# steineggerlab/unicore

Hardware: AMD Instinct MI355X
Metric: 3Di alignments/sec (cluster path) (higher is better)
Workload: dtype u16

## Files before the change

unicore_amd/csrc/uc_sw_pk_impl.hpp:

```cpp
#pragma once
#include <hip/hip_runtime.h>

#include "uc_device.h"
#include "uc_sw_impl.hpp"

namespace uc {

constexpr int SW_PK_OVF = 0x7C00 - 256;

typedef uint16_t u16x2_t __attribute__((ext_vector_type(2)));
typedef uint32_t u32x4_u __attribute__((ext_vector_type(4), aligned(4)));
typedef uint32_t u32x2_u __attribute__((ext_vector_type(2), aligned(4)));
typedef const uint32_t __attribute__((address_space(4))) *sw_cu32p;
__device__ __forceinline__ u16x2_t pk_v(uint32_t x) { return __builtin_bit_cast(u16x2_t, x); }
__device__ __forceinline__ uint32_t pk_u(u16x2_t v) { return __builtin_bit_cast(uint32_t, v); }
__device__ __forceinline__ uint32_t pk_add_sat(uint32_t a, uint32_t b) { return pk_u(__builtin_elementwise_add_sat(pk_v(a), pk_v(b))); }
__device__ __forceinline__ uint32_t pk_sub_sat(uint32_t a, uint32_t b) { return pk_u(__builtin_elementwise_sub_sat(pk_v(a), pk_v(b))); }
__device__ __forceinline__ uint32_t pk_max(uint32_t a, uint32_t b) { return pk_u(__builtin_elementwise_max(pk_v(a), pk_v(b))); }
__device__ __forceinline__ uint32_t pk_min(uint32_t a, uint32_t b) {
    uint32_t r;
    asm("v_pk_min_u16 %0, %1, %2" : "=v"(r) : "v"(a), "v"(b));
    return r;
}
__device__ __forceinline__ uint32_t pk_max3(uint32_t a, uint32_t b, uint32_t c) {
    uint32_t r;
    asm("v_pk_maximum3_f16 %0, %1, %2, %3" : "=v"(r) : "v"(a), "v"(b), "v"(c));
    return r;
}
__device__ __forceinline__ uint32_t pk_max3_s(uint32_t a, uint32_t b, uint32_t c) {
    uint32_t r;
    asm("v_pk_maximum3_f16 %0, %1, %2, %3" : "=v"(r) : "v"(a), "v"(b), "s"(c));
    return r;
}
__device__ __forceinline__ uint32_t pk_max_s(uint32_t a, uint32_t c) {
    uint32_t r;
    asm("v_pk_max_u16 %0, %1, %2" : "=v"(r) : "v"(a), "s"(c));
    return r;
}
__device__ __forceinline__ uint32_t add3_s(uint32_t a, uint32_t b, uint32_t c) {
    uint32_t r;
    asm("v_add3_u32 %0, %1, %2, %3" : "=v"(r) : "v"(a), "v"(b), "s"(c));
    return r;
}
constexpr uint32_t SW_PK_BIAS = 128u * 0x10001u;
constexpr uint32_t SW_PK_UNBIAS = 0u - SW_PK_BIAS;
static_assert(SW_PK_UNBIAS == 0xFF7FFF80u, "the packed -128");

constexpr int SW_MQ_SLOTS = 128;

template <int G, int R, int MODE, int NW, int K = 1>
__global__ void __launch_bounds__(NW * 64) sw_pk_kernel(const SwArgs a) {
    constexpr bool TBB = MODE == 7;
    constexpr uint32_t HB = TBB ? 0u : SW_PK_BIAS;
    constexpr bool KNOWN = MODE == 4 || MODE == 6;
    constexpr int BASE = KNOWN ? MODE - 4 : (TBB ? 0 : MODE);
    constexpr bool TRACK = BASE != 1 && !TBB, MASK = BASE == 2 || TBB, REVQ = BASE != 0, REVT = BASE == 2;
    constexpr int RW = (R + 3) / 4, BW = RW | 1, RSW = G * BW, NT = NW * 64;
    static_assert(R % 2 == 0 && R <= 32, "R must be even, <= 32");
    extern __shared__ __attribute__((aligned(16))) uint32_t lds[];
    static_assert(K == 1 || (K <= 4 && G < 64 && !TBB), "several tasks per workgroup: G < 64, not MODE 7");
    constexpr int PB = 2 * SW_NLET * RSW;
    uint32_t *P3 = lds, *PA = lds + SW_NLET * RSW;
    uint32_t *slot_ctr = lds + K * PB;
    [[maybe_unused]] uint32_t *tinfo = slot_ctr + 4, *sstep = tinfo + 4 * K;
    [[maybe_unused]] uint8_t *stab = (uint8_t *)(sstep + SW_MQ_SLOTS);

    const SwTask task = a.tasks[K * blockIdx.x];
    const int tid = threadIdx.x, lane = tid & 63;
    const int g = lane % G;
    const uint32_t qoff = a.db.off[task.q];
    const int lq = (int)a.db.len[task.q];
    const uint32_t open2 = (uint32_t)a.open * 0x10001u, ext2 = (uint32_t)a.ext * 0x10001u, bias2 = 128u * 0x10001u;
    const uint32_t nslots = (task.count + 1) >> 1;

    for (int idx = tid; idx < SW_NLET * G * RW; idx += NT) {
        const int c = idx / (G * RW), rem = idx % (G * RW), gg = rem / RW, k = rem % RW;
        uint32_t w3 = 0, wa = 0;
#pragma unroll
        for (int b = 0; b < 4; b++) {
            const int row = gg * R + 4 * k + b;
            if (row < lq && c < 21 && 4 * k + b < R) {
                const int qi = REVQ ? lq - 1 - row : row;
                const int q3 = a.db.s3[qoff + qi], qa = a.db.sa[qoff + qi];
                w3 |= (uint32_t)(a.db.S3[q3 * 21 + c] + 64) << (8 * b);
                wa |= (uint32_t)(a.db.SA[qa * 21 + c] + 64) << (8 * b);
            }
        }
        P3[c * RSW + gg * BW + k] = w3;
        PA[c * RSW + gg * BW + k] = wa;
    }
    if constexpr (K > 1) {
        const uint32_t task0 = (uint32_t)K * blockIdx.x, nk = min((uint32_t)K, a.n_tasks - task0);
        uint32_t base[K + 1];
        base[0] = 0; base[1] = nslots;
        if (tid == 0) { tinfo[0] = task.begin; tinfo[1] = task.count; tinfo[2] = (uint32_t)lq; }
#pragma unroll
        for (int t = 1; t < K; t++) {
            base[t + 1] = base[t];
            if ((uint32_t)t < nk) {
                const SwTask tk = a.tasks[task0 + t];
                const uint32_t qofft = a.db.off[tk.q];
                const int lqt = (int)a.db.len[tk.q];
                for (int idx = tid; idx < SW_NLET * G * RW; idx += NT) {
                    const int c = idx / (G * RW), rem = idx % (G * RW), gg = rem / RW, k = rem % RW;
                    uint32_t w3 = 0, wa = 0;
#pragma unroll
                    for (int b = 0; b < 4; b++) {
                        const int row = gg * R + 4 * k + b;
                        if (row < lqt && c < 21 && 4 * k + b < R) {
                            const int qi = REVQ ? lqt - 1 - row : row;
                            const int q3 = a.db.s3[qofft + qi], qa = a.db.sa[qofft + qi];
                            w3 |= (uint32_t)(a.db.S3[q3 * 21 + c] + 64) << (8 * b);
                            wa |= (uint32_t)(a.db.SA[qa * 21 + c] + 64) << (8 * b);
                        }
                    }
                    P3[t * PB + c * RSW + gg * BW + k] = w3;
                    PA[t * PB + c * RSW + gg * BW + k] = wa;
                }
                base[t + 1] += (tk.count + 1) >> 1;
                if (tid == 0) { tinfo[4 * t] = tk.begin; tinfo[4 * t + 1] = tk.count; tinfo[4 * t + 2] = (uint32_t)lqt; }
            }
        }
        const uint32_t mq_slots = min(base[K], (uint32_t)SW_MQ_SLOTS);
        if (tid == 0) tinfo[3] = mq_slots;
        for (uint32_t e = tid; e < mq_slots; e += NT) {
            uint32_t t = 0;
#pragma unroll
            for (int j = 1; j < K; j++) t += e >= base[j] ? 1u : 0u;
            uint32_t eb = 0;
#pragma unroll
            for (int j = 1; j < K; j++) eb = t == (uint32_t)j ? base[j] : eb;
            const SwTask tk = a.tasks[task0 + t];
            const uint32_t i = e - eb, pA = tk.begin + 2 * i, pB = pA + (2 * i + 1 < tk.count ? 1u : 0u);
            const int la = REVT ? a.pte[pA] + 1 : (int)a.db.len[a.pt[pA]], lb = REVT ? a.pte[pB] + 1 : (int)a.db.len[a.pt[pB]];
            sstep[e] = ((uint32_t)((max(la, lb) + G) & ~1) << 8) | (t << 6) | i;
        }
    }
    if (tid == 0) *slot_ctr = 0;
    __syncthreads();
    if constexpr (K > 1) {
        const uint32_t mq_slots = tinfo[3];
        for (uint32_t e = tid; e < mq_slots; e += NT) {
            const uint32_t v = sstep[e], s = v >> 8;
            uint32_t rank = 0;
            for (uint32_t j = 0; j < mq_slots; j++) {
                const uint32_t sj = sstep[j] >> 8;
                rank += (sj > s || (sj == s && j < e)) ? 1u : 0u;
            }
            stab[rank] = (uint8_t)(v & 0xffu);
        }
        __syncthreads();
    }

    uint32_t H[R], E[R], rowbest[(TRACK && !KNOWN) ? R : 1];
    uint32_t mskA[MASK ? RW : 1], mskB[MASK ? RW : 1];
    uint32_t best = HB, Hlast = HB, prevHup = HB, fout = 0;
    int colA = -1, colB = -1;
    [[maybe_unused]] uint32_t knownA = 0, knownB = 0;
    [[maybe_unused]] int key2A = 0x7fffffff, key2B = 0x7fffffff;
    uint32_t gA = 0, gB = 0, toffA = 0, toffB = 0;
    [[maybe_unused]] unsigned long long tbA = 0, tbB = 0;
    [[maybe_unused]] int tsaA = 0, tsbA = 0, tsaB = 0, tsbB = 0;
    [[maybe_unused]] uint32_t trowA = 0, trowB = 0, tslotA = 0, tslotB = 0;
    int tlenA = 0, tlenB = 0, rowoffA = 0, rowoffB = 0;
    bool vB = false, active = false;
    int lst = 0, nst = 0;
    uint32_t c1 = 0, cin = 0;
    struct RawLetters { uint32_t a3, aa, b3, ba; } r2 = {0, 0, 0, 0};
    uint32_t nA3[RW], nAa[RW], nB3[RW], nBa[RW];
    [[maybe_unused]] const uint16_t *ltA = nullptr, *ltB = nullptr;

    auto issue_letters = [&](int st) -> RawLetters {
        RawLetters r;
        if constexpr (G == 64) {
            const int ia = max(min(st, tlenA - 1), 0), ib = max(min(st, tlenB - 1), 0);
            const uint32_t pa = toffA + (uint32_t)(REVT ? max(tlenA - 1 - ia, 0) : ia);
            const uint32_t pb_ = toffB + (uint32_t)(REVT ? max(tlenB - 1 - ib, 0) : ib);
            auto ld = [&](const uint8_t *base, uint32_t p) -> uint32_t {
                const sw_cu32p w = (sw_cu32p)(uintptr_t)(base + (p & ~3u));
                return (*w >> (8u * (p & 3u))) & 0xffu;
            };
            r.a3 = ld(a.db.s3, pa); r.aa = ld(a.db.sa, pa); r.b3 = ld(a.db.s3, pb_); r.ba = ld(a.db.sa, pb_);
        } else {
            const uint32_t ia = REVT ? (uint32_t)max(tlenA - st, 0) : (uint32_t)min(st, tlenA);
            const uint32_t ib = REVT ? (uint32_t)max(tlenB - st, 0) : (uint32_t)min(st, tlenB);
            r.a3 = ltA[ia]; r.b3 = ltB[ib];
            r.aa = 0; r.ba = 0;
        }
        return r;
    };
    auto pack_letters = [&](const RawLetters &r, int st) -> uint32_t {
        if constexpr (G == 64) {
            const uint32_t ca_ = st < tlenA ? (r.a3 | (r.aa << 8)) : SW_PADPACK;
            const uint32_t cb_ = st < tlenB ? (r.b3 | (r.ba << 8)) : SW_PADPACK;
            return ca_ | (cb_ << 16);
        } else if constexpr (TBB) {
            return (st < tlenA ? r.a3 : SW_PADPACK) | ((st < tlenB ? r.b3 : SW_PADPACK) << 16);
        } else {
            return r.a3 | (r.b3 << 16);
        }
    };
    uint32_t off3 = (uint32_t)(g * BW) * 4u, offa = (uint32_t)(SW_NLET * RSW + g * BW) * 4u;
    asm volatile("" : "+v"(off3), "+v"(offa));
    auto fetch_profile = [&]() __attribute__((always_inline)) {
        const char *l8 = (const char *)lds;
        const uint32_t *pA3 = (const uint32_t *)(l8 + (cin & 0xff) * (RSW * 4) + off3), *pAa = (const uint32_t *)(l8 + ((cin >> 8) & 0xff) * (RSW * 4) + offa);
        const uint32_t *pB3 = (const uint32_t *)(l8 + ((cin >> 16) & 0xff) * (RSW * 4) + off3), *pBa = (const uint32_t *)(l8 + (cin >> 24) * (RSW * 4) + offa);
#pragma unroll
        for (int k = 0; k < RW; k++) { nA3[k] = pA3[k]; nAa[k] = pAa[k]; nB3[k] = pB3[k]; nBa[k] = pBa[k]; }
    };

    auto start_slot = [&]() {
        uint32_t idx = 0;
        if (g == 0) idx = atomicAdd(slot_ctr, 1u);
        if constexpr (G == 64) idx = (uint32_t)__builtin_amdgcn_readfirstlane((int)idx);
        else idx = (uint32_t)__shfl((int)idx, lane - g, 64);
        if constexpr (K == 1) active = idx < nslots;
        else active = idx < tinfo[3];
        if (!active) return;
        [[maybe_unused]] uint32_t mq_begin = 0, mq_count = 0;
        [[maybe_unused]] int mq_lq = 0;
        if constexpr (K > 1) {
            const uint32_t code = stab[idx], t = code >> 6;
            idx = code & 63u;
            mq_begin = tinfo[4 * t]; mq_count = tinfo[4 * t + 1]; mq_lq = (int)tinfo[4 * t + 2];
            off3 = (t * PB + (uint32_t)(g * BW)) * 4u;
            offa = off3 + (uint32_t)(SW_NLET * RSW) * 4u;
        }
        const uint32_t iA = 2 * idx, iB = iA + 1;
        vB = iB < (K == 1 ? task.count : mq_count);
        gA = (K == 1 ? task.begin : mq_begin) + iA;
        gB = (K == 1 ? task.begin : mq_begin) + (vB ? iB : iA);
        const uint32_t tA = a.pt[gA], tB = a.pt[gB];
        toffA = a.db.off[tA]; toffB = a.db.off[tB];
        tlenA = REVT ? a.pte[gA] + 1 : (int)a.db.len[tA];
        tlenB = vB ? (REVT ? a.pte[gB] + 1 : (int)a.db.len[tB]) : 0;
        if constexpr (TBB) {
            toffA += (uint32_t)a.pts[gA]; toffB += (uint32_t)a.pts[gB];
            tlenA = a.pte[gA] - a.pts[gA] + 1;
            tlenB = vB ? a.pte[gB] - a.pts[gB] + 1 : 0;
            tbA = a.tboff[gA]; tbB = a.tboff[gB];
            const int qsA = a.pqs[gA], qeA = a.pqe[gA], qsB = a.pqs[gB], qeB = a.pqe[gB];
            {
                constexpr int RBc = 4 * RW;
                const TbBand bA = tb_band_of(qsA, qeA, tlenA, G, R, a.tb_band), bB = tb_band_of(qsB, qeB, vB ? tlenB : 1, G, R, a.tb_band);
                const bool fullA = bA.nl >= G, fullB = bB.nl >= G;
                tsaA = fullA ? 0 : g * (R + 1) - bA.dhi; tsbA = fullA ? 0x7fffffff : g * (R + 1) + R - 1 - bA.dlo;
                tsaB = fullB ? 0 : g * (R + 1) - bB.dhi; tsbB = fullB ? 0x7fffffff : g * (R + 1) + R - 1 - bB.dlo;
                trowA = (uint32_t)(bA.nl * RBc); trowB = (uint32_t)(bB.nl * RBc);
                tslotA = (uint32_t)((g % bA.nl) * RBc); tslotB = (uint32_t)((g % bB.nl) * RBc);
            }
#pragma unroll
            for (int k = 0; k < RW; k++) {
                uint32_t ma = 0, mb = 0;
#pragma unroll
                for (int b = 0; b < 4; b++) {
                    const int row = g * R + 4 * k + b;
                    ma |= (row >= qsA && row <= qeA ? 0xFFu : 0u) << (8 * b);
                    mb |= (row >= qsB && row <= qeB ? 0xFFu : 0u) << (8 * b);
                }
                mskA[k] = ma; mskB[k] = mb;
            }
        } else if constexpr (MASK) {
            rowoffA = (K == 1 ? lq : mq_lq) - 1 - a.pqe[gA];
            rowoffB = (K == 1 ? lq : mq_lq) - 1 - a.pqe[gB];
#pragma unroll
            for (int k = 0; k < RW; k++) {
                uint32_t ma = 0, mb = 0;
#pragma unroll
                for (int b = 0; b < 4; b++) {
                    ma |= (g * R + 4 * k + b >= rowoffA ? 0xFFu : 0u) << (8 * b);
                    mb |= (g * R + 4 * k + b >= rowoffB ? 0xFFu : 0u) << (8 * b);
                }
                mskA[k] = ma; mskB[k] = mb;
            }
        }
        if constexpr (G != 64) {
            ltA = a.db.lt + toffA - (REVT ? 1 : 0);
            ltB = vB ? a.db.lt + toffB - (REVT ? 1 : 0) : a.db.lt + toffA - 1;
        }
#pragma unroll
        for (int r = 0; r < R; r++) { H[r] = HB; E[r] = HB; }
        if constexpr (TRACK && !KNOWN) {
#pragma unroll
            for (int r = 0; r < R; r++) rowbest[r] = HB;
        }
        if constexpr (KNOWN) {
            knownA = (uint32_t)a.pscore[gA] + 128u;
            knownB = vB ? (uint32_t)a.pscore[gB] + 128u : 128u;
            key2A = 0x7fffffff; key2B = 0x7fffffff;
        }
        best = HB; colA = -1; colB = -1; Hlast = HB; prevHup = HB; fout = 0;
        lst = 0;
        nst = (max(tlenA, tlenB) + G) & ~1;
        c1 = pack_letters(issue_letters(1), 1);
        r2 = issue_letters(2);
        if constexpr (G == 64) {
            c1 = (uint32_t)__builtin_amdgcn_readfirstlane((int)c1);
            r2.a3 = (uint32_t)__builtin_amdgcn_readfirstlane((int)r2.a3); r2.aa = (uint32_t)__builtin_amdgcn_readfirstlane((int)r2.aa);
            r2.b3 = (uint32_t)__builtin_amdgcn_readfirstlane((int)r2.b3); r2.ba = (uint32_t)__builtin_amdgcn_readfirstlane((int)r2.ba);
        }
        cin = (uint32_t)shift_from_prev_lane<G>((int)(SW_PADPACK * 0x10001u), (int)pack_letters(issue_letters(0), 0), g);
        fetch_profile();
    };

    auto do_step = [&](const int st, const bool ODD) __attribute__((always_inline)) {
        uint32_t sA[RW], sB[RW];
#pragma unroll
        for (int k = 0; k < RW; k++) {
            sA[k] = nA3[k] + nAa[k];
            sB[k] = nB3[k] + nBa[k];
            if constexpr (MASK) { sA[k] &= mskA[k]; sB[k] &= mskB[k]; }
        }
        cin = (uint32_t)shift_from_prev_lane<G>((int)cin, (int)c1, g);
        c1 = pack_letters(r2, st + 2);
        r2 = issue_letters(st + 3);
        fetch_profile();
        const uint32_t Hup = (uint32_t)shift_from_prev_lane_zero<G>((int)Hlast, g);
        uint32_t f = (uint32_t)shift_from_prev_lane_zero<G>((int)fout, g);
        uint32_t diag = prevHup;
        if constexpr (!TBB) diag = pk_max_s(prevHup, HB);
        uint32_t colmax = 0;
        [[maybe_unused]] uint32_t code[TBB ? R : 1];
#pragma unroll
        for (int r = 0; r < R; r++) {
            const uint32_t ub = __builtin_amdgcn_perm(sB[r >> 2], sA[r >> 2], 0x0c000c00u | ((4u + (r & 3)) << 16) | (uint32_t)(r & 3));
            uint32_t x;
            if constexpr (TBB) x = pk_sub_sat(pk_add_sat(diag, ub), bias2);
            else x = add3_s(diag, ub, SW_PK_UNBIAS);
            const uint32_t e = E[r];
            const uint32_t h = pk_max3(x, e, f);
            const uint32_t hprev = H[r];
            diag = hprev;
            H[r] = h;
            const uint32_t t = pk_sub_sat(h, open2);
            const uint32_t esub = pk_sub_sat(e, ext2), fsub = pk_sub_sat(f, ext2);
            if constexpr (TBB) code[r] = h;
            if constexpr (TBB) E[r] = pk_max(esub, t);
            else E[r] = pk_max3_s(esub, t, HB);
            f = pk_max(fsub, t);
            if constexpr (TRACK && !KNOWN) { if (ODD) rowbest[r] = pk_max3(rowbest[r], hprev, h); }
            if (r & 1) colmax = pk_max3(colmax, H[r - 1], h);
        }
        if constexpr (TBB) {
            uint32_t wa[RW], wb[RW];
#pragma unroll
            for (int k = 0; k < RW; k++) {
                const uint32_t c0 = code[4 * k], c1_ = 4 * k + 1 < R ? code[4 * k + 1] : 0u;
                const uint32_t c2 = 4 * k + 2 < R ? code[4 * k + 2] : 0u, c3 = 4 * k + 3 < R ? code[4 * k + 3] : 0u;
                const uint32_t p01 = __builtin_amdgcn_perm(c1_, c0, 0x06020400u);
                const uint32_t p23 = __builtin_amdgcn_perm(c3, c2, 0x06020400u);
                wa[k] = __builtin_amdgcn_perm(p23, p01, 0x05040100u);
                wb[k] = __builtin_amdgcn_perm(p23, p01, 0x07060302u);
            }
            uint8_t *dA = a.tbm + tbA + (unsigned long long)st * trowA + tslotA;
            uint8_t *dB = a.tbm + tbB + (unsigned long long)st * trowB + tslotB;
            auto put = [&](uint8_t *d, const uint32_t *w) __attribute__((always_inline)) {
                int k = 0;
#pragma unroll
                for (; k + 4 <= RW; k += 4) {
                    u32x4_u v = {w[k], w[k + 1], w[k + 2], w[k + 3]};
                    *(u32x4_u *)(d + 4 * k) = v;
                }
#pragma unroll
                for (; k + 2 <= RW; k += 2) {
                    u32x2_u v = {w[k], w[k + 1]};
                    *(u32x2_u *)(d + 4 * k) = v;
                }
#pragma unroll
                for (; k < RW; k++) *(uint32_t *)(d + 4 * k) = w[k];
            };
            if (st >= tsaA && st <= tsbA) put(dA, wa);
            if (vB && st >= tsaB && st <= tsbB) put(dB, wb);
        }
        if constexpr (TRACK && !KNOWN) {
            const uint32_t cmA = colmax & 0xffffu, cmB = colmax >> 16;
            colA = cmA > (best & 0xffffu) ? st - g : colA;
            colB = cmB > (best >> 16) ? st - g : colB;
        }
        if constexpr (KNOWN) {
            const bool evA = knownA != 128u && (colmax & 0xffffu) == knownA;
            const bool evB = knownB != 128u && (colmax >> 16) == knownB;
            if (__builtin_amdgcn_ballot_w64(evA || evB) != 0) {
                if (evA) {
                    int first = 0, cnt = 0;
#pragma unroll
                    for (int r = R - 1; r >= 0; r--) { const bool hit = (H[r] & 0xffffu) == knownA; first = hit ? r : first; cnt += hit ? 1 : 0; }
                    if (colA < 0) colA = ((st - g) << 6) | (first << 1);
                    if constexpr (MODE == 6) colA |= (cnt > 1 || first != ((colA >> 1) & 31)) ? 1 : 0;
                    key2A = min(key2A, ((g * R + first) << 16) | (st - g));
                }
                if (evB) {
                    int first = 0, cnt = 0;
#pragma unroll
                    for (int r = R - 1; r >= 0; r--) { const bool hit = (H[r] >> 16) == knownB; first = hit ? r : first; cnt += hit ? 1 : 0; }
                    if (colB < 0) colB = ((st - g) << 6) | (first << 1);
                    if constexpr (MODE == 6) colB |= (cnt > 1 || first != ((colB >> 1) & 31)) ? 1 : 0;
                    key2B = min(key2B, ((g * R + first) << 16) | (st - g));
                }
            }
        }
        best = pk_max(best, colmax);
        Hlast = H[R - 1];
        fout = f;
        prevHup = Hup;
    };

    auto finish_slot = [&]() {
        if constexpr (TBB) return;
        if constexpr (KNOWN) {
            knownA -= 128u; knownB -= 128u;
#pragma unroll
            for (int half = 0; half < 2; half++) {
                const int st1 = half ? colB : colA, col = st1 >> 6, row = (st1 >> 1) & 31;
                int key = st1 < 0 ? 0x7fffffff : ((col << 11) | (g * R + row));
                int nrows = st1 < 0 ? 0 : 1 + ((st1 & 1) ? G : 0);
                int key2 = half ? key2B : key2A;
#pragma unroll
                for (int m = 1; m < G; m <<= 1) {
                    key = min(key, __shfl_xor(key, m, 64));
                    nrows += __shfl_xor(nrows, m, 64);
                    key2 = min(key2, __shfl_xor(key2, m, 64));
                }
                const bool valid = half ? vB : true;
                const uint32_t gp = half ? gB : gA;
                if (g == 0 && valid) {
                    const int rowoff = half ? rowoffB : rowoffA;
                    const bool found = key != 0x7fffffff;
                    a.oscore[gp] = (int)(half ? knownB : knownA);
                    a.oqe[gp] = found ? (key & 2047) - rowoff : -2;
                    a.ote[gp] = found ? ((key >> 11) | ((MODE == 6 && nrows == 1) ? SW_TE_UNIQUE : 0)) : -2;
                    if (a.oqe2) {
                        a.oqe2[gp] = found ? (key2 >> 16) - rowoff : -2;
                        a.ote2[gp] = found ? (key2 & 0xffff) : -2;
                    }
                }
            }
            return;
        }
#pragma unroll
        for (int half = 0; half < 2; half++) {
            int score = half ? (int)(best >> 16) : (int)(best & 0xffffu);
            int col = half ? colB : colA;
#pragma unroll
            for (int m = 1; m < G; m <<= 1) {
                const int os = __shfl_xor(score, m, 64), oc = __shfl_xor(col, m, 64);
                const bool take = os > score || (os == score && oc < col);
                score = take ? os : score;
                col = take ? oc : col;
            }
            int cnt = 0, minrow = 1 << 30;
            if constexpr (TRACK) {
#pragma unroll
                for (int r = R - 1; r >= 0; r--) {
                    const int rb = half ? (int)(rowbest[r] >> 16) : (int)(rowbest[r] & 0xffffu);
                    if (rb == score) { cnt++; minrow = g * R + r; }
                }
#pragma unroll
                for (int m = 1; m < G; m <<= 1) {
                    cnt += __shfl_xor(cnt, m, 64);
                    minrow = min(minrow, __shfl_xor(minrow, m, 64));
                }
            }
            const bool valid = half ? vB : true;
            const uint32_t gp = half ? gB : gA;
            if (g == 0 && valid) {
                const int sc = score - 128;
                a.oscore[gp] = sc;
                if constexpr (TRACK) {
                    const int rowoff = half ? rowoffB : rowoffA;
                    int qe = -1, te = -1;
                    if (sc > 0) { te = col; qe = (cnt == 1 && sc < SW_PK_OVF) ? minrow - rowoff : -2; }
                    a.oqe[gp] = qe;
                    a.ote[gp] = te;
                }
            }
        }
    };

    start_slot();
    while (__builtin_amdgcn_ballot_w64(active) != 0) {
        if (active) {
            do_step(lst, false);
            do_step(lst + 1, true);
            lst += 2;
            if (lst >= nst) {
                finish_slot();
                start_slot();
            }
        }
    }
}

constexpr int sw_pk_class_queries(int G, int R, int mode) {
    if (G != 16 || R < 4) return 1;
    if (mode == 4) return (R == 8 || R == 10 || R == 14) ? 1 : 2;
    return (mode == 0 || mode == 1 || mode == 6) ? 2 : 1;
}

template <int MODE>
int launch_sw_pk_class_mode(int G, int R, const SwArgs &a, uint32_t n_tasks, hipStream_t s, int kmax, uint32_t tcap) {
#define UC_SW_LAUNCH(GG, RR, NW, KK)                                                                    \
    {                                                                                                   \
        const size_t lds = (size_t)KK * 2 * SW_NLET * GG * BW * 4 + 16 + (KK > 1 ? 16 * KK + 5 * SW_MQ_SLOTS : 0); \
        static PerDeviceOnce once;                                                                      \
        if (lds > 64 * 1024)                                                                            \
            once([&] { (void)hipFuncSetAttribute((const void *)sw_pk_kernel<GG, RR, MODE, NW, KK>,       \
                                                 hipFuncAttributeMaxDynamicSharedMemorySize, (int)lds); }); \
        SwArgs ak = a;                                                                                  \
        ak.n_tasks = n_tasks;                                                                           \
        hipLaunchKernelGGL((sw_pk_kernel<GG, RR, MODE, NW, KK>), dim3((n_tasks + KK - 1) / KK), dim3(NW * 64), lds, s, ak); \
        return KK;                                                                                      \
    }
#define UC_SW_CASE(GG, RR)                                                                              \
    if (G == GG && R == RR) {                                                                           \
        constexpr int BW = (((RR + 3) / 4) | 1);                                                        \
         \
        constexpr int NW = GG == 16 ? 2 : (GG == 32 ? 4 : (RR < 14 ? 2 : 8));                           \
        constexpr int KC = sw_pk_class_queries(GG, RR, MODE);                                           \
        if constexpr (KC > 1) {                                                                         \
            const uint32_t ts = (tcap + 1) / 2;                             \
             \
            if (kmax > 1 && ts <= 64 && KC * ts <= (uint32_t)SW_MQ_SLOTS) UC_SW_LAUNCH(GG, RR, NW * KC, KC) \
        }                                                                                               \
        UC_SW_LAUNCH(GG, RR, NW, 1)                                                                     \
    }
    UC_SW_CASE(16, 2) UC_SW_CASE(16, 4) UC_SW_CASE(16, 6) UC_SW_CASE(16, 8) UC_SW_CASE(16, 10) UC_SW_CASE(16, 12)
    UC_SW_CASE(16, 14) UC_SW_CASE(16, 16) UC_SW_CASE(16, 18) UC_SW_CASE(16, 20) UC_SW_CASE(16, 22) UC_SW_CASE(16, 24)
    UC_SW_CASE(32, 14) UC_SW_CASE(32, 16) UC_SW_CASE(32, 18) UC_SW_CASE(32, 20) UC_SW_CASE(32, 22) UC_SW_CASE(32, 24)
    UC_SW_CASE(64, 14) UC_SW_CASE(64, 16) UC_SW_CASE(64, 18) UC_SW_CASE(64, 20) UC_SW_CASE(64, 22) UC_SW_CASE(64, 24)
    UC_SW_CASE(64, 26) UC_SW_CASE(64, 28) UC_SW_CASE(64, 30) UC_SW_CASE(64, 32)
    if constexpr (MODE == 4 || MODE == 6) {
        UC_SW_CASE(64, 2) UC_SW_CASE(64, 4) UC_SW_CASE(64, 6) UC_SW_CASE(64, 8) UC_SW_CASE(64, 10) UC_SW_CASE(64, 12)
    }
#undef UC_SW_CASE
#undef UC_SW_LAUNCH
    fprintf(stderr, "unicore-cluster: no packed SW kernel for class (G=%d, R=%d)\n", G, R);
    abort();
}

template <int MODE>
void preload_sw_pk_mode() {
    hipFuncAttributes fa;
    (void)hipFuncGetAttributes(&fa, (const void *)sw_pk_kernel<64, 14, MODE, 8>);
}

}
```

Before: 25.45 million.

## Load letter pairs as 32-bit words and track best column via packed age counter

For the non-64-group, non-TBB path, the letter stream is now loaded two columns at a time as 32-bit words, with the two lanes' letters combined by byte permute. This halves the per-step global loads and index arithmetic. The per-column best-column tracking is replaced by a packed u16 'age since last improvement' counter, updated with saturated subtract and packed multiply-add, and the column is reconstructed at the end. This removes two compares and selects per step, at the cost of relying on 16-bit age arithmetic and unaligned reads in the reverse-target case.

```diff
diff --git a/unicore_amd/csrc/uc_sw_pk_impl.hpp b/unicore_amd/csrc/uc_sw_pk_impl.hpp
--- a/unicore_amd/csrc/uc_sw_pk_impl.hpp
+++ b/unicore_amd/csrc/uc_sw_pk_impl.hpp
@@ -40,6 +40,11 @@
 __device__ __forceinline__ uint32_t add3_s(uint32_t a, uint32_t b, uint32_t c) {
     uint32_t r;
     asm("v_add3_u32 %0, %1, %2, %3" : "=v"(r) : "v"(a), "v"(b), "s"(c));
+    return r;
+}
+__device__ __forceinline__ uint32_t pk_mad(uint32_t a, uint32_t b, uint32_t c) {
+    uint32_t r;
+    asm("v_pk_mad_u16 %0, %1, %2, %3" : "=v"(r) : "v"(a), "v"(b), "v"(c));
     return r;
 }
 constexpr uint32_t SW_PK_BIAS = 128u * 0x10001u;
@@ -156,6 +161,7 @@
     uint32_t mskA[MASK ? RW : 1], mskB[MASK ? RW : 1];
     uint32_t best = HB, Hlast = HB, prevHup = HB, fout = 0;
     int colA = -1, colB = -1;
+    [[maybe_unused]] uint32_t age2 = 0;
     [[maybe_unused]] uint32_t knownA = 0, knownB = 0;
     [[maybe_unused]] int key2A = 0x7fffffff, key2B = 0x7fffffff;
     uint32_t gA = 0, gB = 0, toffA = 0, toffB = 0;
@@ -169,6 +175,17 @@
     struct RawLetters { uint32_t a3, aa, b3, ba; } r2 = {0, 0, 0, 0};
     uint32_t nA3[RW], nAa[RW], nB3[RW], nBa[RW];
     [[maybe_unused]] const uint16_t *ltA = nullptr, *ltB = nullptr;
+    constexpr bool LT2 = G != 64 && !TBB;
+    constexpr uint32_t LT2_FIRST = REVT ? 0x07060302u : 0x05040100u, LT2_SECOND = REVT ? 0x05040100u : 0x07060302u;
+    [[maybe_unused]] uint32_t wA = 0, wB = 0;
+    [[maybe_unused]] int clA = 0, clB = 0;
+    typedef uint32_t __attribute__((aligned(2))) lt2_word;
+    auto issue_words = [&](int c) __attribute__((always_inline)) {
+        const uint32_t ia = REVT ? (uint32_t)max(clA - c, 0) : (uint32_t)min(c, clA);
+        const uint32_t ib = REVT ? (uint32_t)max(clB - c, 0) : (uint32_t)min(c, clB);
+        if constexpr (REVT) { wA = *(const lt2_word *)(ltA + ia); wB = *(const lt2_word *)(ltB + ib); }
+        else { wA = *(const uint32_t *)(ltA + ia); wB = *(const uint32_t *)(ltB + ib); }
+    };
 
     auto issue_letters = [&](int st) -> RawLetters {
         RawLetters r;
@@ -182,8 +199,7 @@
             };
             r.a3 = ld(a.db.s3, pa); r.aa = ld(a.db.sa, pa); r.b3 = ld(a.db.s3, pb_); r.ba = ld(a.db.sa, pb_);
         } else {
-            const uint32_t ia = REVT ? (uint32_t)max(tlenA - st, 0) : (uint32_t)min(st, tlenA);
-            const uint32_t ib = REVT ? (uint32_t)max(tlenB - st, 0) : (uint32_t)min(st, tlenB);
+            const uint32_t ia = (uint32_t)min(st, tlenA), ib = (uint32_t)min(st, tlenB);
             r.a3 = ltA[ia]; r.b3 = ltB[ib];
             r.aa = 0; r.ba = 0;
         }
@@ -275,9 +291,14 @@
                 mskA[k] = ma; mskB[k] = mb;
             }
         }
-        if constexpr (G != 64) {
-            ltA = a.db.lt + toffA - (REVT ? 1 : 0);
-            ltB = vB ? a.db.lt + toffB - (REVT ? 1 : 0) : a.db.lt + toffA - 1;
+        if constexpr (LT2) {
+            ltA = a.db.lt + toffA - (REVT ? 2 : 0);
+            ltB = vB ? a.db.lt + toffB - (REVT ? 2 : 0) : a.db.lt + toffA - 2;
+            clA = REVT ? tlenA : (tlenA + 1) & ~1;
+            clB = REVT ? tlenB : (tlenB + 1) & ~1;
+        } else if constexpr (G != 64) {
+            ltA = a.db.lt + toffA;
+            ltB = vB ? a.db.lt + toffB : a.db.lt + toffA - 1;
         }
 #pragma unroll
         for (int r = 0; r < R; r++) { H[r] = HB; E[r] = HB; }
@@ -290,9 +311,18 @@
             knownB = vB ? (uint32_t)a.pscore[gB] + 128u : 128u;
             key2A = 0x7fffffff; key2B = 0x7fffffff;
         }
-        best = HB; colA = -1; colB = -1; Hlast = HB; prevHup = HB; fout = 0;
+        best = HB; colA = -1; colB = -1; age2 = 0; Hlast = HB; prevHup = HB; fout = 0;
         lst = 0;
         nst = (max(tlenA, tlenB) + G) & ~1;
+        if constexpr (LT2) {
+            issue_words(0);
+            const uint32_t c0 = __builtin_amdgcn_perm(wB, wA, LT2_FIRST);
+            c1 = __builtin_amdgcn_perm(wB, wA, LT2_SECOND);
+            issue_words(2);
+            cin = (uint32_t)shift_from_prev_lane<G>((int)(SW_PADPACK * 0x10001u), (int)c0, g);
+            fetch_profile();
+            return;
+        }
         c1 = pack_letters(issue_letters(1), 1);
         r2 = issue_letters(2);
         if constexpr (G == 64) {
@@ -313,8 +343,13 @@
             if constexpr (MASK) { sA[k] &= mskA[k]; sB[k] &= mskB[k]; }
         }
         cin = (uint32_t)shift_from_prev_lane<G>((int)cin, (int)c1, g);
-        c1 = pack_letters(r2, st + 2);
-        r2 = issue_letters(st + 3);
+        if constexpr (LT2) {
+            c1 = __builtin_amdgcn_perm(wB, wA, ODD ? LT2_SECOND : LT2_FIRST);
+            if (ODD) issue_words(st + 3);
+        } else {
+            c1 = pack_letters(r2, st + 2);
+            r2 = issue_letters(st + 3);
+        }
         fetch_profile();
         const uint32_t Hup = (uint32_t)shift_from_prev_lane_zero<G>((int)Hlast, g);
         uint32_t f = (uint32_t)shift_from_prev_lane_zero<G>((int)fout, g);
@@ -374,9 +409,9 @@
             if (vB && st >= tsaB && st <= tsbB) put(dB, wb);
         }
         if constexpr (TRACK && !KNOWN) {
-            const uint32_t cmA = colmax & 0xffffu, cmB = colmax >> 16;
-            colA = cmA > (best & 0xffffu) ? st - g : colA;
-            colB = cmB > (best >> 16) ? st - g : colB;
+            const uint32_t d = pk_sub_sat(colmax, best);
+            const uint32_t nm = pk_sub_sat(0x00010001u, d);
+            age2 = pk_mad(age2, nm, nm);
         }
         if constexpr (KNOWN) {
             const bool evA = knownA != 128u && (colmax & 0xffffu) == knownA;
@@ -441,7 +476,8 @@
 #pragma unroll
         for (int half = 0; half < 2; half++) {
             int score = half ? (int)(best >> 16) : (int)(best & 0xffffu);
-            int col = half ? colB : colA;
+            int col = -1;
+            if constexpr (TRACK) col = (int)(((uint32_t)(nst - 1 - g) - (half ? age2 >> 16 : age2)) & 0xffffu);
 #pragma unroll
             for (int m = 1; m < G; m <<= 1) {
                 const int os = __shfl_xor(score, m, 64), oc = __shfl_xor(col, m, 64);
```

Result: faster. 25.91 million (median of 6 runs) (+1.8%).
